# AbbVie-ComputationalGenomics/SAIGEgds

Hardware: AMD Instinct MI355X
Metric: variants/sec seqAssocGLMM_SPA at N=430K; achieved HBM GB/s vs roofline (higher is better)
Workload: dtype f64

## Files before the change

### saigegds_amd/csrc/host_init.h

```cpp
extern "C" const char *sgx_version(void) { return "saigehip 0.1 (gfx950)"; }
extern "C" const char *sgx_last_error(void) { return g_err.c_str(); }

extern "C" int sgx_device_count(void)
{
	int n = 0;
	if (hipGetDeviceCount(&n) != hipSuccess) return 0;
	return n;
}

extern "C" size_t sgx_row_stride(int32_t n_samp)
{
	return (size_t)((n_samp + 511) / 512) * 128;
}

static double thr_or(double v, double dflt) { return std::isfinite(v) ? v : dflt; }

extern "C" int sgx_set_thresholds(sgx_handle *h, double maf, double mac, double missing,
	double spa_pval)
{
	if (!h) return fail(SGX_EINVAL, "sgx_set_thresholds: NULL handle");
	h->md.thr_maf = thr_or(maf, -1);
	h->md.thr_mac = thr_or(mac, -1);
	h->md.thr_missing = thr_or(missing, 1);
	h->md.thr_spa = thr_or(spa_pval, 0.05);
// ... 61 lines not shown
			worst = std::max(worst, fabsl(t - (LD)m->t_XVX_inv_XV[(size_t)i * K + k]));
			scale = std::max(scale, fabsl((LD)m->t_XVX_inv_XV[(size_t)i * K + k]));
		}
	}
	if (!(worst <= 1e-13L * scale)) return false;
	for (int a = 0; a < K; a++)
		for (int b = 0; b < K; b++) out[(size_t)b * K + a] = (double)M[(size_t)a * K + b];
	for (int a = 0; a < K * K; a++) if (!std::isfinite(out[a])) return false;
	return true;
}

static int alloc_workspace(sgx_handle *h)
{
	const int N = h->md.N;
	{
		int least = 0, greatest = 0;
		HIPCHK(hipDeviceGetStreamPriorityRange(&least, &greatest));
		HIPCHK(h->stream.create(hipStreamNonBlocking, least));
		HIPCHK(h->hstream.create(hipStreamNonBlocking, greatest));
		HIPCHK(h->s3_side.create(hipStreamNonBlocking, greatest));
	}
	HIPCHK(h->s3_fork.create(hipEventDisableTiming));
	HIPCHK(h->s3_join.create(hipEventDisableTiming));
	HIPCHK(h->counters.alloc(24));
	HIPCHK(h->h_counters.alloc(24));
	for (DevEvent &e : h->ev) HIPCHK(e.create());
	for (DevEvent &e : h->evk) HIPCHK(e.create());
	HIPCHK(h->ev_lists.create());
	hipDeviceProp_t prop;
	HIPCHK(hipGetDeviceProperties(&prop, h->device));
	h->spa_grid = prop.multiProcessorCount * 2;
	h->n_cu = prop.multiProcessorCount;
	h->scratch_stride = 2 * (((size_t)N + 63) & ~(size_t)63);
	HIPCHK(h->scratch.alloc(h->scratch_stride * h->spa_grid));
	if (!h->md.quant) {
		h->nwg5 = ((size_t)((N + 63) / 64) * 16 <= 32 * 1024) ? h->n_cu * 4 : h->n_cu;
		HIPCHK(h->scr5.alloc((size_t)h->nwg5 * spa5_wg_bytes(N)));
		HIPCHK(h->cur5.alloc(8));
	}
	return SGX_OK;
}

static int check_model_consistency(const sgx_model *m)
{
	const int N = m->n_samp, K = m->n_coeff;
	if (!m->t_XXVX_inv || !m->XV)
		return fail(SGX_EINVAL, "sgx_init: SAIGEHIP_CHECK_MODEL needs t_XXVX_inv and XV");
	for (int i = 0; i < N; i++) {
		const double *x = m->t_X + (size_t)i * K, *xv = m->XV + (size_t)i * K,
			*a = m->t_XXVX_inv + (size_t)i * K, *av = m->t_XVX_inv_XV + (size_t)i * K;
		int k0 = 0;
		double sx = 0, sa = 0;
		for (int k = 0; k < K; k++) {
			if (std::fabs(x[k]) > std::fabs(x[k0])) k0 = k;
			sx = std::max(sx, std::fabs(xv[k])); sa = std::max(sa, std::fabs(av[k]));
		}
		if (x[k0] == 0) continue;
		const double V = xv[k0] / x[k0];
		for (int k = 0; k < K; k++) {
			if (std::fabs(xv[k] - V * x[k]) > 1e-8 * sx)
				return fail(SGX_EINVAL, "sgx_init: XV[%d,%d] = %g is not V t_X = %g", k, i, xv[k], V * x[k]);
			if (std::fabs(av[k] - V * a[k]) > 1e-8 * sa)
// ... 183 lines not shown
{
	if (!h) return;
	(void)hipSetDevice(h->device);
	for (hipStream_t st : {(hipStream_t)h->stream, (hipStream_t)h->s3_side, (hipStream_t)h->hstream}) if (st) (void)hipStreamSynchronize(st);
	for (sgx_handle *t : h->twins) sgx_free(t);
	for (sgx_block *b : h->tmp_blk) sgx_block_free(b);
	delete h;
}

static int ensure_recs(sgx_handle *h, size_t n)
{
	if (3 * n <= h->recs.cap) return SGX_OK;
	HIPCHK(hipStreamSynchronize(h->stream));
	HIPCHK(h->recs.release());
	int rc = grow(h->fallback, n);
	if (!rc && !h->md.quant) {
		h->nseg = (h->md.N + spa_seg(h->md.K) - 1) / spa_seg(h->md.K);
		rc = grow(h->fb_spa2, n);
		if (!rc) rc = grow(h->fb_x2, n);
		h->vcap4 = (int)std::min<size_t>(n, 65536);
		h->nround4 = (int)((n + h->vcap4 - 1) / h->vcap4);
		if (!rc) rc = grow(h->seg4, (size_t)h->nseg * SPA4_NSMAX * h->vcap4);
	}
	if (!rc && h->mf_ok) rc = grow(h->mf_acc, n * (size_t)(2 * h->mfe.acc_stride - 16));
	if (!rc) rc = grow(h->recs, 3 * n);
	return rc;
}
```

### saigegds_amd/csrc/host_scan.h

```cpp

template <typename T>
static int ensure_buf(sgx_handle *lane, DevBuf<T> &buf, size_t need)
{
	if (need <= buf.cap) return SGX_OK;
	for (hipStream_t st : {(hipStream_t)lane->stream, (hipStream_t)lane->hstream, (hipStream_t)lane->s3_side}) if (st) HIPCHK(hipStreamSynchronize(st));
	return grow(buf, need);
}

struct S3Shape { int nbf, naf, nc, nla, nlb, da, db; };
#define S3_SHAPE(...) S3Shape{__VA_ARGS__},
static constexpr S3Shape s3_shapes[2][15] = {{S3_FOR_EACH_NBF(S3_SHAPE)}, {S3_FOR_EACH_NBF_MISS(S3_SHAPE)}};
#undef S3_SHAPE

template <bool MISS, int I>
static int launch_score3(sgx_handle *h, const sgx_block *b, RowsRef rr, size_t M, int grid, int slots, S3Plan &pl)
{
	constexpr S3Shape s = s3_shapes[MISS][I];
	hipStream_t st = h->hstream;
	pl = s3_plan(M, b->ntile, grid, s.naf * s.nc, rr.bpv);
	int rc = ensure_buf(h, h->s3_slabs, (size_t)pl.ng * pl.ipg * s.nc * s.naf * slots * 256);
	if (rc) return rc;
	const size_t lds = s3_lds_bytes(s.nbf, s.naf, s.nc, s.da, s.db);
	auto kern = score3_kernel<s.nbf, s.naf, s.nc, s.nla, s.nlb, s.da, s.db, MISS>;
	bool &attr = (MISS ? h->s3_attr_miss : h->s3_attr)[s.nbf];
// ... 39 lines not shown
			const unsigned chunks = (unsigned)((M + 4 * tpw - 1) / (4 * tpw));
			hipLaunchKernelGGL(s3_t3_kernel<decltype(pp)::value>, dim3(chunks * (unsigned)b->nr), dim3(256), 0, h->s3_side,
				(int)M, md.P, h->dQ, L, h->s3_t3);
		});
		HIPCHK(hipGetLastError());
		HIPCHK(hipEventRecord(h->s3_join, h->s3_side));
		HIPCHK(hipStreamWaitEvent(st, h->s3_join, 0));
	}
	const bool miss = form == FORM_THREE;
	const int NBF = h->mf_nbfv[0] + 1;
	const int slots = miss ? 2 * NBF - 1 : NBF;
	const int grid = std::max(8, h->n_cu & ~7);
	constexpr int NSHAPE = (int)(sizeof s3_shapes[0] / sizeof s3_shapes[0][0]);
	int i = 0;
	while (i < NSHAPE && s3_shapes[miss][i].nbf != NBF) i++;
	S3Plan pl{};
	const auto shapes = std::make_integer_sequence<int, NSHAPE>();
	const bool found = miss ? with_int<0>(i, [&](auto I) { rc = launch_score3<true, decltype(I)::value>(h, b, rr, M, grid, slots, pl); }, shapes)
		: with_int<0>(i, [&](auto I) { rc = launch_score3<false, decltype(I)::value>(h, b, rr, M, grid, slots, pl); }, shapes);
	if (!found) return fail(SGX_EINVAL, "score3: %d B fragments not supported", NBF);
	if (rc) return rc;
	HIPCHK(hipGetLastError());
	const S3Shape &sh = s3_shapes[miss][i];
	const int acc_stride = 16 * slots;
	const int per = sh.nc * sh.naf * slots * 256;
	hipLaunchKernelGGL(s3_reduce_kernel, dim3((unsigned)((per / 4 + 255) / 256), (unsigned)pl.vt), dim3(256), 0, st,
		pl, (int)M, sh.nc, sh.naf, slots, h->s3_slabs, h->mf_acc, acc_stride, h->counters, h->cur5);
	const int btop = md.quant ? 0 : (int)(2 * M);
	if (!with_k(md.K, [&](auto kk) {
		constexpr int KK = decltype(kk)::value;
		hipLaunchKernelGGL((score3_epilogue<KK>), dim3((unsigned)((M + s3e_vb(KK) - 1) / s3e_vb(KK))), dim3(s3e_vb(KK)), 0, st,
			(int)M, md, h->mfe, h->mf_acc, acc_stride, miss ? 16 * NBF : 0, h->s3_t3, b->nr, L.lcnt, L.ld, h->s3_ovf, h->recs,
			h->counters, btop, h->fb_spa2, h->fb_x2, out8, valid, h->guard_tol);
		hipLaunchKernelGGL((score2b_kernel<2 * KK + 2, 256>), dim3((unsigned)std::min<size_t>(M, 4 * (size_t)h->n_cu)), dim3(256), 0, st,
			rr, (int)M, md, h->recs, h->counters, out8, valid, (const int *)h->s3_ovf, 23, btop, h->fb_spa2, h->fb_x2);
	}))
		return fail(SGX_EINVAL, "score3: unsupported K=%d", md.K);
	HIPCHK(hipGetLastError());
	return scan_end<IN_2BIT>(h, st, b, rr, M, out8, lazy_dense);
}

static int next_lane(sgx_handle *h, size_t M, sgx_handle **lane_out)
{
	sgx_handle *lane = h, *other = nullptr;
	if (h->n_lanes > 1) {
		lane = h->next_lane ? h->twins[h->next_lane - 1] : h;
		other = h->last_issued;
		h->next_lane = (h->next_lane + 1) % h->n_lanes;
	}
	int rc = sync_lane(lane);
	if (rc) return rc;
	h->last_issued = lane;
	rc = ensure_recs(lane, M);
	if (rc) return rc;
	if (other && other != lane && other->stats_pending) HIPCHK(hipStreamWaitEvent(lane->hstream, other->ev[1], 0));
	*lane_out = lane;
	return SGX_OK;
}

static int scan_form(const sgx_handle *lane, const sgx_block *b, ScanForm *form)
{
	const sgx_handle *p = lane->owner ? lane->owner : lane;
// ... 77 lines not shown
```

### saigegds_amd/csrc/host_spa.h

```cpp


template <int LO, typename F, int... I>
static bool with_int(int v, F &&f, std::integer_sequence<int, I...>)
{
	return ((v == LO + I && (f(std::integral_constant<int, LO + I>()), true)) || ...);
}
template <typename F>
static bool with_k(int K, F &&f) { return with_int<1>(K, f, std::make_integer_sequence<int, KMAX>()); }
template <typename F>
static void with_pp(int P, F &&f)
{
	if (P <= 8) f(std::integral_constant<int, 8>());
	else if (P <= 16) f(std::integral_constant<int, 16>());
	else if (P <= 32) f(std::integral_constant<int, 32>());
	else f(std::integral_constant<int, 64>());
}

static dim3 mf_grid(int n_cu, size_t rows, int ntile, int *tps, int vpb = MF_VPB, int wg_per_cu = 2)
{
	const int vt = (int)((rows + vpb - 1) / vpb);
	int sk = std::max(1, (n_cu * wg_per_cu * 4 + vt / 2) / vt);
	sk = std::min(sk, std::max(1, ntile / 24));
	if (sk >= 6) sk = (sk + 7) & ~7;
	sk = std::min(sk, std::max(1, ntile / 2));
	*tps = (ntile + sk - 1) / sk;
	*tps += *tps & 1;
	sk = (ntile + *tps - 1) / *tps;
	return dim3((unsigned)vt, (unsigned)sk);
}

template <int KK, int NCX, int INPUT>
static const void *spa4_moments_fn()
{
	if constexpr (INPUT == IN_2BIT) return (const void *)spa4_moments<KK, NCX>;
	else return (const void *)spa4_moments_ds<KK, NCX, INPUT>;
}

template <int KK, int INPUT>
static void launch_dense(sgx_handle *h, RowsRef rr, size_t M, int slot, const int *list, double *out8)
{
	const dim3 sgrid((unsigned)std::min<size_t>(M, (size_t)h->spa_grid));
	hipLaunchKernelGGL((spa_kernel<KK, 512, INPUT>), sgrid, dim3(512), 0, h->stream, rr,
		h->md, h->recs, h->counters, slot, list, h->scratch, h->scratch_stride, out8);
}

template <int KK, int INPUT>
static int launch_spa_k(sgx_handle *h, RowsRef rr, size_t M, double *out8, bool lazy_dense)
{
	const DevModel &md = h->md;
	hipStream_t st = h->stream;
	if (h->force_v1 && INPUT != IN_2BIT) {
		launch_dense<KK, INPUT>(h, rr, M, 0, nullptr, out8);
		return SGX_OK;
	}
	const size_t fl = spa4_lds_bytes(KK);
	if (!h->mom_attr_set[INPUT]) {
		HIPCHK(hipFuncSetAttribute(spa4_moments_fn<KK, SPA4_NCA, INPUT>(), hipFuncAttributeMaxDynamicSharedMemorySize, (int)fl));
		HIPCHK(hipFuncSetAttribute(spa4_moments_fn<KK, SPA4_NCB, INPUT>(), hipFuncAttributeMaxDynamicSharedMemorySize, (int)fl));
		h->mom_attr_set[INPUT] = true;
	}
	const int nround = (int)((M + h->vcap4 - 1) / h->vcap4);
	const int btop = (int)(2 * M);
	const dim3 gsolve((unsigned)std::min((h->vcap4 + 3) / 4, 4 * h->n_cu));
	const size_t rowb5 = (size_t)((md.N + 63) / 64) * 16;
	const size_t l5 = (INPUT == IN_2BIT && rowb5 <= 120 * 1024) ? rowb5 : 0;
	const bool small5 = INPUT == IN_2BIT && rowb5 <= 32 * 1024;
	if (l5 > 48 * 1024 && !h->spa5_attr_set[INPUT]) {
		HIPCHK(hipFuncSetAttribute((const void *)spa5_kernel<KK, INPUT, 0, 512>, hipFuncAttributeMaxDynamicSharedMemorySize, (int)l5));
		HIPCHK(hipFuncSetAttribute((const void *)spa5_kernel<KK, INPUT, 1, 512>, hipFuncAttributeMaxDynamicSharedMemorySize, (int)l5));
		h->spa5_attr_set[INPUT] = true;
	}
	auto moments = [&](auto ncx, int tier, int rd) {
		constexpr int NCX = decltype(ncx)::value;
		if constexpr (INPUT == IN_2BIT)
			hipLaunchKernelGGL((spa4_moments<KK, NCX>), dim3((unsigned)h->n_cu), dim3(WAVE * spa4_waves(KK)), fl, st, rr, md, h->nseg,
				tier, btop, rd * h->vcap4, h->vcap4, h->recs, h->counters, h->seg4, h->cur5 + 2);
		else
			hipLaunchKernelGGL((spa4_moments_ds<KK, NCX, INPUT>), dim3((unsigned)h->n_cu), dim3(WAVE * spa4_waves(KK)), fl, st,
				(const void *)rr.base, rr.bpv, md, h->nseg, tier, btop, rd * h->vcap4, h->vcap4, h->recs, h->counters, h->seg4, h->cur5 + 2);
		hipLaunchKernelGGL((spa4_solve<KK, NCX>), gsolve, dim3(256), 0, st, md, h->nseg, tier, btop, rd * h->vcap4, h->vcap4,
			h->recs, h->counters, h->seg4, h->fallback, h->fb_x2, out8, h->force_dense ? 1 : 0, h->force_exact ? 1 : 0);
	};
	for (int rd = 0; rd < nround; rd++) moments(std::integral_constant<int, SPA4_NCA>(), 0, rd);
	for (int rd = 0; rd < nround; rd++) moments(std::integral_constant<int, SPA4_NCB>(), 1, rd);
	const size_t ws5 = spa5_wg_bytes(md.N);
	auto spa5 = [&](auto threads, int nwg) {
		constexpr int T5 = decltype(threads)::value;
		if constexpr (T5 == 512 || INPUT == IN_2BIT) {
			hipLaunchKernelGGL((spa5_kernel<KK, INPUT, 0, T5>), dim3((unsigned)nwg), dim3(T5), l5, st, rr, md, h->recs, h->counters,
				h->fb_spa2, h->fb_x2, h->cur5, h->fallback, h->scr5, out8, h->force_dense ? 1 : 0, h->force_exact ? 1 : 0, l5,
				h->spa_scan_rows, ws5, 3);
			hipLaunchKernelGGL((spa5_kernel<KK, INPUT, 1, T5>), dim3((unsigned)nwg), dim3(T5), l5, st, rr, md, h->recs, h->counters,
				h->fb_x2, h->fb_x2, h->cur5 + 1, h->fallback, h->scr5, out8, h->force_dense ? 1 : 0, h->force_exact ? 1 : 0, l5,
				h->spa_scan_rows, ws5, 4);
		}
	};
	if (small5) spa5(std::integral_constant<int, 128>(), h->nwg5);
	else spa5(std::integral_constant<int, 512>(), h->n_cu);
	if (!lazy_dense) launch_dense<KK, INPUT>(h, rr, M, 2, h->fallback, out8);
	return SGX_OK;
}

template <int INPUT>
static int launch_spa(sgx_handle *h, RowsRef rr, size_t M, double *out8, bool lazy_dense = false)
{
	h->stats.spa_launches = 0;
	if (h->md.quant) return SGX_OK;
	int rc = SGX_OK;
	with_k(h->md.K, [&](auto kk) { rc = launch_spa_k<decltype(kk)::value, INPUT>(h, rr, M, out8, lazy_dense); });
	if (rc) return rc;
	HIPCHK(hipGetLastError());
	const bool v1 = h->force_v1 && INPUT != IN_2BIT;
	h->stats.spa_launches = v1 ? 1u : (uint32_t)(4 * ((M + h->vcap4 - 1) / h->vcap4) + 3);
	if (lazy_dense && !v1) { h->pend_dense.active = true; h->pend_dense.rr = rr; h->pend_dense.M = M; h->pend_dense.out8 = out8; }
	return SGX_OK;
}

static int launch_pending_dense(sgx_handle *h)
{
	with_k(h->md.K, [&](auto kk) {
		launch_dense<decltype(kk)::value, IN_2BIT>(h, h->pend_dense.rr, h->pend_dense.M, 2, h->fallback, h->pend_dense.out8);
	});
	HIPCHK(hipGetLastError());
	return SGX_OK;
}

static int scan_begin(sgx_handle *h, hipStream_t sst, ScanForm form, const sgx_block *b)
{
	h->form = form;
	if (b) HIPCHK(hipStreamWaitEvent(sst, b->ready, 0));
	if (form == FORM_FP64) {
		HIPCHK(hipMemsetAsync(h->counters, 0, 24 * sizeof(int), sst));
		if (h->cur5) HIPCHK(hipMemsetAsync(h->cur5, 0, 8 * sizeof(int), sst));
	}
	HIPCHK(hipEventRecord(h->ev[0], sst));
	return SGX_OK;
}

template <int INPUT>
static int scan_end(sgx_handle *h, hipStream_t sst, const sgx_block *b, RowsRef rr, size_t M, double *out8, bool lazy_dense)
{
	HIPCHK(hipEventRecord(h->ev[1], sst));
	h->stats.score_launches = h->form == FORM_FP64 ? 1 : 5;
	if (sst != h->stream) HIPCHK(hipStreamWaitEvent(h->stream, h->ev[1], 0));
	int rc = launch_spa<INPUT>(h, rr, M, out8, lazy_dense);
	if (rc) return rc;
	if (lazy_dense) h->pend_dense.blk = b;
	HIPCHK(hipEventRecord(h->ev[2], h->stream));
	if (b) {
		HIPCHK(hipEventRecord(b->last_read, h->stream));
		const_cast<sgx_block *>(b)->was_read = true;
	}
	HIPCHK(hipMemcpyAsync(h->h_counters, h->counters, 24 * sizeof(int), hipMemcpyDeviceToHost, h->stream));
	h->stats.n_variants = M;
	h->stats_pending = true;
	return SGX_OK;
}
// ... 51 lines not shown
```

### saigegds_amd/csrc/host_state.h

```cpp

struct sgx_block {
	int device = 0;
	int N = 0, ntile = 0, nr = 1;
	size_t cap = 0;
	size_t M = 0;
	bool lists_only = false;
	DevEvent ready;
	DevEvent last_read;
	bool was_read = false;
	DevBuf<uint8_t> rows;
	size_t bpv = 0;
	const uint8_t *ext_rows = nullptr; size_t ext_bpv = 0;
	DevBuf<unsigned> idx; size_t idx_cap = 0;
	DevBuf<unsigned> cursor;
	DevBuf<unsigned> lstart;
	DevBuf<int> lcnt;
	DevBuf<int> nzp, n2p;
	DevBuf<int> n3;
	DevBuf<uint8_t> ovf;
	DevBuf<int> nzv, n2v;
	DevBuf<unsigned> cptr;
	DevBuf<unsigned> cidx;
	size_t cidx_cap = 0;
	DevBuf<uint8_t> corient;
// ... 13 lines not shown
	DevStream stream;
	DevStream hstream;
	DevStream s3_side;
	DevStream cstream;
	DevEvent s3_fork, s3_join;
	DevEvent ev[3];
	DevEvent evk[2];
	DevEvent ev_lists;
	DevEvent ev_h2d;
	DevEvent ev_copy[2];
	DevEvent ev_done[2];
	struct { DevBuf<double> F, X, y, mu, mu2, XM; DevBuf<uint8_t> Fl; DevBuf<long long> Q; } model;
	DevModel md{};
	DevBuf<SpaRec> recs;
	DevBuf<int> fallback;
	DevBuf<int> fb_spa2;
	DevBuf<int> fb_x2;
	int nseg = 0;
	bool force_dense = false;
	DevBuf<double> seg4;
	int vcap4 = 0, nround4 = 0;
	bool spa5_attr_set[3] = {false, false, false};
	bool mom_attr_set[3] = {false, false, false};
	DevBuf<uint8_t> scr5; DevBuf<int> cur5; int nwg5 = 0;
	bool spa_scan_rows = false;
	bool force_exact = false;
	bool mf_ok = false;
	MfTab mf[MF_MAXG]{};
	int mf_nbfv[MF_MAXG]{};
	MfEpi mfe{};
	const long long *dQ = nullptr;
	DevBuf<int> mf_acc;
	DevBuf<int> s3_slabs;
	DevBuf<long long> s3_t3;
	DevBuf<int> s3_ovf;
	bool s3_attr[17] = {false};
	bool s3_attr_miss[17] = {false};
	sgx_block *tmp_blk[2] = {nullptr, nullptr};
	int n_cu = 256;
	DevBuf<int> counters;
	PinBuf<int> h_counters;
	DevBuf<double> scratch; size_t scratch_stride = 0; int spa_grid = 0;
	DevBuf<uint8_t> stage_in;
	size_t pipe_bytes = 0;
	DevBuf<uint8_t> pipe_in[2];
	DevBuf<uint8_t> pipe_raw[2];
	DevBuf<uint8_t> pipe_pk[2];
	DevBuf<int> pipe_flag; PinBuf<int> h_pipe_flag;
	DevBuf<int> pk_sel;
	DevBuf<unsigned> db2_row0;
	DevBuf<double> pipe_out[2]; DevBuf<uint8_t> pipe_valid[2];
	PinBuf<double> pin_out[2]; PinBuf<uint8_t> pin_valid[2];
	DevBuf<uint8_t> stage_pk;
	DevBuf<double> ds_part;
	DevBuf<double> skat_part;
	DevBuf<double> skat_fin;
	DevBuf<double> stage_out; DevBuf<uint8_t> stage_valid;
	DevBuf<double> skk_A, skk_Y, skk_XZ, skk_cpart, skk_cs;
	DevBuf<SkkTile> skk_tiles;
	double skk_ms[3] = {0, 0, 0};
	DevBuf<double> ckm_set;
	int ckm_n = 0;
	sgx_kmat *ckm_km = nullptr;
	std::vector<double> ckm_D, ckm_q, ckm_Einv, ckm_w;
	std::vector<uint8_t> ckm_bad;
	bool ckm_eok = false;
	double ckm_tau[2] = {0, 0}, ckm_tol = 0;
	int ckm_maxiter = 0;
	DevBuf<double> cond_B;
	DevBuf<double> cond_ce;
	int n_cond = 0;
	DevBuf<double> cond_part, cond_fin;
	DevBuf<uint8_t> firth_scr;
	DevBuf<double> eig_A, eig_out, eig_scr;
	DevBuf<int> eig_sw;
	DevBuf<uint8_t> eig_meta;
	bool eig_attr_set = false;
	bool evk_set = false;
	bool lists_timed = false;
	sgx_stats stats{};
	bool force_v1 = false;
	bool stats_pending = false;
	struct { bool active = false; RowsRef rr{}; size_t M = 0; double *out8 = nullptr; const sgx_block *blk = nullptr; } pend_dense;
	sgx_handle *twins[3] = {nullptr, nullptr, nullptr};
	int n_lanes = 1;
	sgx_handle *owner = nullptr;
	bool dense_mode = false;
	int dense_opt = -1;
	double guard_tol = 2e-11;
	ScanForm form = FORM_FP64;
	int next_lane = 0;
	sgx_handle *last_issued = nullptr;
	sgx_stats total{};
	uint64_t total_calls = 0;
};

#define SGX_DENSE_ON  0.005
#define SGX_DENSE_OFF 0.003

static int set_dev(sgx_handle *h)
{
	HIPCHK(hipSetDevice(h->device));
	return SGX_OK;
}
```

### saigegds_amd/csrc/kern_score.h

```cpp
#pragma once


template <int P, int BLOCK>
__global__ void __launch_bounds__(BLOCK)
score2b_kernel(RowsRef rr, int M, DevModel md,
	SpaRec *__restrict__ recs, int *__restrict__ counters, double *__restrict__ out8,
	uint8_t *__restrict__ valid, const int *__restrict__ list, int list_counter, int btop, int *__restrict__ fb_series, int *__restrict__ fb_exact)
{
	__shared__ double sh[P * (BLOCK / WAVE)];
	__shared__ int shi[3 * (BLOCK / WAVE)];
	const int nwork = list ? counters[list_counter] : M;
	for (int wi = blockIdx.x; wi < nwork; wi += gridDim.x) {
	const int j = list ? list[wi] : wi;
	const int N = md.N, tid = threadIdx.x;
	const int lane = tid & (WAVE - 1), wid = tid / WAVE;
	constexpr int NW = BLOCK / WAVE;
	const int nvec = (N + 63) >> 6;
	auto row_piece = [&](int v) -> uint4 { return *reinterpret_cast<const uint4 *>(rr.base + rr_piece(rr, (size_t)j, (size_t)v)); };
	__syncthreads();

	int n1 = 0, n2 = 0, n3 = 0;
	for (int v = tid; v < nvec; v += BLOCK) {
		const uint4 q = row_piece(v);
		const uint32_t ww[4] = {q.x, q.y, q.z, q.w};
#pragma unroll
		for (int d = 0; d < 4; d++) {
			const uint32_t w = ww[d] & keep_mask(N - (v * 64 + d * 16));
			const uint32_t lo = w & LO_MASK, hi = (w >> 1) & LO_MASK;
			n3 += __popc(lo & hi);
			n1 += __popc(lo & ~hi);
			n2 += __popc(hi & ~lo);
		}
	}
	n1 = wave_sum_i(n1); n2 = wave_sum_i(n2); n3 = wave_sum_i(n3);
	if (lane == 0) { shi[wid] = n1; shi[NW + wid] = n2; shi[2 * NW + wid] = n3; }
	__syncthreads();
	n1 = n2 = n3 = 0;
#pragma unroll
	for (int w = 0; w < NW; w++) { n1 += shi[w]; n2 += shi[NW + w]; n3 += shi[2 * NW + w]; }

	const VarHead h = make_head(md, double(n1 + 2 * n2), N - n3);
	if (!h.pass) {
		if (tid == 0) { nan_row(out8 + (size_t)j * 8); valid[j] = 0; }
		continue;
	}

	double acc[P];
#pragma unroll
	for (int a = 0; a < P; a++) acc[a] = 0;
	const uint32_t zx = h.minus ? 0xAAAAAAAAu : 0u;
	const double *__restrict__ F = md.F;
	for (int v = tid; v < nvec; v += BLOCK) {
		const uint4 q = row_piece(v);
		const uint32_t ww[4] = {q.x, q.y, q.z, q.w};
#pragma unroll
		for (int d = 0; d < 4; d++) {
			const int base = v * 64 + d * 16;
			const uint32_t km = keep_mask(N - base);
			const uint32_t w = ww[d];
			uint32_t nz = nz_fields((w ^ zx) & km) ;
			while (nz) {
				const int b = __ffs(nz) - 1;
				nz &= nz - 1;
				const double g = sel4(h.lut, (w >> b) & 3u);
				const double *f = F + (size_t)(base + (b >> 1)) * P;
#pragma unroll
				for (int a = 0; a < P - 2; a += 2) {
					const double2 t = *reinterpret_cast<const double2 *>(f + a);
					acc[a] = fma(g, t.x, acc[a]);
					acc[a + 1] = fma(g, t.y, acc[a + 1]);
				}
				const double2 t = *reinterpret_cast<const double2 *>(f + P - 2);
				acc[P - 2] = fma(g, t.x, acc[P - 2]);
				acc[P - 1] = fma(g * g, t.y, acc[P - 1]);
			}
		}
	}
	block_sum<P, BLOCK>(acc, sh);

	if (tid == 0) {
		double *o = out8 + (size_t)j * 8;
		double cbuf[KMAX], pn, Ssc, v2sc;
		valid[j] = 1;
		if (score_epilogue<(P - 2) / 2>(md, h, acc, o, cbuf, &pn, &Ssc, &v2sc)) {
			spa_push<(P - 2) / 2>(md, recs, counters, btop, fb_series, fb_exact, j, h.minus, h.minus ? (2 * h.Num - h.AC) : h.AC,
				h.minus ? (N - n2) : (n1 + n2 + n3), h.lut, pn, Ssc, v2sc, cbuf);
		}
		atomicAdd(&counters[1], 1);
	}
	}
}


template <typename T> __device__ __forceinline__ bool ds_missing(T v);
template <> __device__ __forceinline__ bool ds_missing<uint8_t>(uint8_t v) { return v == 0xFF; }
template <> __device__ __forceinline__ bool ds_missing<double>(double v) { return !isfinite(v); }

template <int P, int BLOCK, typename T>
__global__ void __launch_bounds__(BLOCK)
score_ds_kernel(const T *__restrict__ ds, int M, DevModel md, SpaRec *__restrict__ recs,
	int *__restrict__ counters, double *__restrict__ out8, uint8_t *__restrict__ valid)
{
	__shared__ double sh[P * (BLOCK / WAVE)];
	const int j = blockIdx.x;
	if (j >= M) return;
	const int N = md.N, tid = threadIdx.x;
	const T *row = ds + (size_t)j * N;

	double hd[2] = {0, 0};
	for (int i = tid; i < N; i += BLOCK) {
		const T v = row[i];
		if (!ds_missing<T>(v)) { hd[0] += (double)v; hd[1] += 1.0; }
	}
// ... 157 lines not shown
```

### saigegds_amd/csrc/kern_score3.h

```cpp
#pragma once
#include <type_traits>

#ifndef S3_V4I_DEFINED
#define S3_V4I_DEFINED
typedef int s3_v4i __attribute__((ext_vector_type(4)));
#endif

#include "s3_layout.h"

template <int OFF> __device__ __forceinline__ void s3_ds_read(s3_v4i &dst, uint32_t addr)
{
	asm volatile("ds_read_b128 %0, %1 offset:%2" : "=v"(dst) : "v"(addr), "n"(OFF));
}
template <int N> __device__ __forceinline__ void s3_lgkm_wait(s3_v4i &reg) { asm volatile("s_waitcnt lgkmcnt(%1)" : "+v"(reg) : "n"(N)); }
__device__ __forceinline__ void s3_tie(s3_v4i &reg) { asm volatile("" : "+v"(reg)); }
template <int N, int CNT> __device__ __forceinline__ void s3_wait_regs(s3_v4i *regs)
{
	s3_lgkm_wait<N>(regs[0]);
#pragma unroll
	for (int i = 1; i < CNT; i++) s3_tie(regs[i]);
}

template <int I, int N, typename F>
__device__ __forceinline__ void s3_static_for(F &&f)
// ... 507 lines not shown
		for (int k = 0; k < NB; k++) mine[k] = (e + k * PP + c < e1) ? idx[e + k * PP + c] : 0xFFFFFFFFu;
		constexpr int UN = PP <= 16 ? 8 : 4;
		constexpr int UNR = PP <= 16 ? 2 : 1;
#pragma unroll
		for (int k = 0; k < NB; k++)
#pragma unroll UNR
			for (int j0 = 0; j0 < PP; j0 += UN) {
				long long q[UN];
#pragma unroll
				for (int j = 0; j < UN; j++) {
					const unsigned s = (unsigned)__shfl((int)mine[k], gbase + j0 + j, 64);
					q[j] = (s != 0xFFFFFFFFu && c < P) ? Q[(size_t)s * P + c] : 0;
				}
#pragma unroll
				for (int j = 0; j < UN; j++) { hi += q[j] >> 32; lo += q[j] & 0xFFFFFFFFll; }
			}
	}
	if (v < M && c < P) {
		long long *o = part + (((size_t)g * M + v) * P + c) * 2;
		o[0] = hi; o[1] = lo;
	}
}

__global__ void __launch_bounds__(256)
s3_reduce_kernel(S3Plan pl, int M, int NC, int NAF, int NBF, const int *__restrict__ slabs, int *__restrict__ accbuf, int stride,
	int *__restrict__ counters, int *__restrict__ cursors)
{
	if (blockIdx.x == 0 && blockIdx.y == 0 && threadIdx.x < 32) {
		if (threadIdx.x < 24) counters[threadIdx.x] = 0;
		if (threadIdx.x < 8 && cursors) cursors[threadIdx.x] = 0;
	}
	const int e = (blockIdx.x * 256 + threadIdx.x) * 4, per = NC * NAF * NBF * 256, vtile = blockIdx.y;
	if (e >= per) return;
	const int lane = e & 63, reg = (e >> 6) & 3, fb = e >> 8;
	const int b = fb % NBF, wf = fb / NBF;
	const int v = (vtile * pl.fpw + wf) * 16 + (lane >> 4) * 4 + reg;
	if (v >= M) return;
	s3_v4i sum = (s3_v4i){0, 0, 0, 0};
	for (int g = 0; g < pl.ng; g++) {
		int first, count;
		s3_items_of(pl, vtile, g, first, count);
		for (int id = first; id < first + count; id++) sum += *reinterpret_cast<const s3_v4i *>(slabs + (size_t)id * per + e);
	}
	*reinterpret_cast<s3_v4i *>(accbuf + (size_t)v * stride + b * 16 + (lane & 15)) = sum;
}

__host__ __device__ constexpr int s3e_vb(int K) { return K <= 8 ? 256 : 128; }
template <int K>
__global__ void __launch_bounds__(256)
score3_epilogue(int M, DevModel md, MfEpi ep, const int *__restrict__ accbuf, int acc_stride, int miss_off,
	const long long *__restrict__ t3part , int nr,
	const int *__restrict__ lcnt , size_t ld, int *__restrict__ ovf_list,
	SpaRec *__restrict__ recs, int *__restrict__ counters, int btop, int *__restrict__ fb_series, int *__restrict__ fb_exact,
	double *__restrict__ out8, uint8_t *__restrict__ valid, double guard_tol)
{
	constexpr int P = 2 * K + 2, CW = P - 1;
	constexpr int S3E_VB = s3e_vb(K);
	__shared__ double s_acc[S3E_VB][P | 1];
	__shared__ double s_imp[S3E_VB];
	__shared__ int s_n[S3E_VB][4];
	__shared__ long long s_ftot[P][2];
	__shared__ int s_col[P][3];
	const int tid = threadIdx.x, j0 = blockIdx.x * S3E_VB;
	const int N = md.N;
	for (int c = tid; c < P; c += S3E_VB) {
		s_col[c][0] = ep.ccol[c]; s_col[c][1] = ep.climb[c]; s_col[c][2] = ep.escale[c];
		s_ftot[c][0] = ep.ftot_hi[c]; s_ftot[c][1] = ep.ftot_lo[c];
	}
	{
		const int j = j0 + tid;
		const int *a0 = accbuf + (size_t)min(j, M - 1) * acc_stride;
		int n3 = 0;
		bool over = false;
		if (miss_off) n3 = a0[miss_off + ep.col_ones] / 4;
		else {
			for (int g0 = 0; g0 < nr; g0 += 8) {
				int cn[8];
#pragma unroll
				for (int u = 0; u < 8; u++) cn[u] = lcnt[(size_t)min(g0 + u, nr - 1) * ld + min(j, M - 1)];
#pragma unroll
				for (int u = 0; u < 8; u++) if (g0 + u < nr) { over |= cn[u] < 0; n3 += cn[u] < 0 ? 0 : cn[u]; }
			}
		}
		if (j >= M) n3 = 0;
		{
			const int tot = wave_total_i(n3);
			if ((tid & 63) == 0 && tot >= 64) atomicAdd(&counters[22], tot >> 6);
		}
		int state = 0, n1 = 0, n2 = 0;
		double imp = 0;
		if (j < M) {
			if (over) ovf_list[atomicAdd(&counters[23], 1)] = j;
			else {
				const long long AC = (long long)(a0[ep.col_ones] / 4) - 3ll * n3;
				n2 = a0[ep.col_b1 + ep.climb[CW]] / 8 - n3;
				n1 = (int)(AC - 2ll * n2);
				const VarHead h = make_head(md, (double)AC, N - n3);
				if (!h.pass) { nan_row(out8 + (size_t)j * 8); valid[j] = 0; }
				else { state = h.minus ? 2 : 1; imp = 2 * h.AF; }
			}
		}
		s_n[tid][0] = n1; s_n[tid][1] = n2; s_n[tid][2] = n3; s_n[tid][3] = state;
		s_imp[tid] = imp;
	}
	__syncthreads();
	for (int task = tid; task < S3E_VB * P; task += S3E_VB) {
		const int vl = task / P, c = task - vl * P, j = j0 + vl;
		const int state = s_n[vl][3];
		if (!state) continue;
		const int cc = s_col[c][0], nl = s_col[c][1];
		if (nl == 0) { s_acc[vl][c] = 0; continue; }
		const int *a0 = accbuf + (size_t)j * acc_stride;
		const bool minus = state == 2;
		const double imp = s_imp[vl];
		int lv[MF_NLIMB], lm[MF_NLIMB], lb[MF_NLIMB];
#pragma unroll
		for (int l = 0; l < MF_NLIMB; l++) lv[l] = a0[cc + min(l, nl - 1)];
		HiLo T3 = hl(0, 0);
		if (miss_off) {
#pragma unroll
			for (int l = 0; l < MF_NLIMB; l++) lm[l] = a0[miss_off + cc + min(l, nl - 1)];
		} else {
			const long long *p = t3part + ((size_t)j * P + c) * 2;
			const size_t gs = (size_t)M * P * 2;
			for (int g0 = 0; g0 < nr; g0 += 8) {
				long long ph[8], pl[8];
#pragma unroll
				for (int u = 0; u < 8; u++) { const long long *q = p + (size_t)min(g0 + u, nr - 1) * gs; ph[u] = q[0]; pl[u] = q[1]; }
#pragma unroll
				for (int u = 0; u < 8; u++) if (g0 + u < nr) { T3.hi += ph[u]; T3.lo += pl[u]; }
			}
		}
		if (c == CW) {
#pragma unroll
			for (int l = 0; l < MF_NLIMB; l++) lb[l] = a0[ep.col_b1 + min(l, nl - 1)];
		}
		auto limbs = [&](const int (&x)[MF_NLIMB]) -> HiLo {
			long long lo = 0, hi = 0;
#pragma unroll
			for (int l = 3; l >= 0; l--) lo = lo * 256 + (l < nl ? x[l] : 0);
#pragma unroll
			for (int l = MF_NLIMB - 1; l >= 4; l--) hi = hi * 256 + (l < nl ? x[l] : 0);
			return hl(hi, lo);
		};
		const HiLo V = limbs(lv);
		if (miss_off) T3 = limbs(lm);
		const HiLo W = hl_axpy(-3, T3, V);
		const double t3d = hl_to_double(T3);
		double r;
		if (c != CW) {
			double sm;
			if (!minus) sm = hl_to_double(W) + imp * t3d;
			else sm = hl_to_double(hl(2 * s_ftot[c][0] - W.hi, 2 * s_ftot[c][1] - W.lo)) - imp * t3d;
			r = ldexp(sm, -s_col[c][2]);
		} else {
			const HiLo B2 = limbs(lb);
			const HiLo H2 = hl(B2.hi / 2 - T3.hi, B2.lo / 2 - T3.lo);
			double w;
			if (!minus) {
				w = hl_to_double(hl_axpy(2, H2, W)) + imp * imp * t3d;
			} else {
				const HiLo S1 = hl_axpy(-2, H2, W);
				const HiLo R = hl(s_ftot[CW][0] - S1.hi - H2.hi - T3.hi, s_ftot[CW][1] - S1.lo - H2.lo - T3.lo);
				w = hl_to_double(hl_axpy(4, R, S1)) + (2 - imp) * (2 - imp) * t3d;
			}
			r = ldexp(w, -s_col[CW][2]);
		}
		s_acc[vl][c] = r;
	}
	__syncthreads();
	const int j = j0 + tid;
	if (j >= M || !s_n[tid][3]) return;
	const int n1 = s_n[tid][0], n2 = s_n[tid][1], n3 = s_n[tid][2];
	const long long AC = (long long)n1 + 2ll * n2;
	const VarHead h = make_head(md, (double)AC, N - n3);
	const double imp = 2 * h.AF;
	double *o = out8 + (size_t)j * 8;
	double acc[P];
#pragma unroll
	for (int c = 0; c < P; c++) acc[c] = s_acc[tid][c];
	if (ep.derive_c) {
#pragma unroll
		for (int x = 0; x < K; x++) {
			double cx = 0;
#pragma unroll
			for (int y = 0; y < K; y++) cx = fma(ep.XVXi[x * K + y], acc[K + y], cx);
			acc[x] = cx;
		}
	}
	{
		const double g2 = (double)n1 + 4.0 * n2 + (h.minus ? (2 - imp) * (2 - imp) : imp * imp) * n3;
		const double spread = 8.0 * sqrt(fmax(g2, 1.0));
		double dcol[P];
#pragma unroll
		for (int c = 0; c < P; c++) dcol[c] = (ep.climb[c] && !(md.quant && c == CW)) ? spread * ldexp(1.0, -ep.escale[c]) : 0.0;
// ... 6 lines not shown
			sat[y] = t;
		}
		double dquad = 0, dec = 0, dS = dcol[2 * K], quad = 0, ec = 0, sac = 0;
#pragma unroll
		for (int a = 0; a < K; a++) {
			double t = 0;
#pragma unroll
			for (int b = 0; b < K; b++) t = fma(md.XVX[a * K + b], acc[b], t);
			quad = fma(t, acc[a], quad);
			dquad += 2 * dcol[a] * fabs(t - acc[K + a]);
			ec = fma(acc[K + a], acc[a], ec);
			dec += dcol[K + a] * fabs(acc[a]);
			sac = fma(md.S_a[a], acc[a], sac);
			dS += ep.derive_c ? fabs(sat[a]) * dcol[K + a] : fabs(md.S_a[a]) * dcol[a];
		}
		const double var2 = quad + acc[CW] - 2 * ec, S = acc[2 * K] - sac;
		const double dvar = dquad + 2 * dec + dcol[CW];
		const double sd = sqrt(md.r * fmax(var2, 0.0) * (md.quant ? 1.0 / fmax(h.mac, 1.0) : 1.0)) * (md.quant ? md.tau0 * sqrt(fmax(h.mac, 1.0)) : 1.0);
		const double z = fabs(S) / sd;
		const double dz = dS / sd + 0.5 * z * dvar / var2;
		if (!(dz * fmax(1.0, z) <= guard_tol)) {
			ovf_list[atomicAdd(&counters[23], 1)] = j;
			atomicAdd(&counters[21], 1);
			return;
		}
	}
	double cbuf[KMAX], pn, Ssc, v2sc;
	valid[j] = 1;
	if (score_epilogue<(P - 2) / 2>(md, h, acc, o, cbuf, &pn, &Ssc, &v2sc)) {
		spa_push<K>(md, recs, counters, btop, fb_series, fb_exact, j, h.minus, h.minus ? (2 * h.Num - h.AC) : h.AC,
			h.minus ? (N - n2) : (n1 + n2 + n3), h.lut, pn, Ssc, v2sc, cbuf);
	}
	{
		const unsigned long long act = __ballot(true);
		if (__builtin_amdgcn_mbcnt_hi((uint32_t)(act >> 32), __builtin_amdgcn_mbcnt_lo((uint32_t)act, 0u)) == 0u) atomicAdd(&counters[1], (int)__popcll(act));
	}
}
#endif
```

Baseline: 18.51 million.

## Fuse slab reduction, epilogue and overflow fallback into one score3 tail kernel

```diff
diff --git a/saigegds_amd/csrc/host_init.h b/saigegds_amd/csrc/host_init.h
--- a/saigegds_amd/csrc/host_init.h
+++ b/saigegds_amd/csrc/host_init.h
@@ -107,7 +107,9 @@
 	}
 	HIPCHK(h->s3_fork.create(hipEventDisableTiming));
 	HIPCHK(h->s3_join.create(hipEventDisableTiming));
-	HIPCHK(h->counters.alloc(24));
+	HIPCHK(h->cnt_sets.alloc(2 * 24));
+	HIPCHK(hipMemsetAsync(h->cnt_sets, 0, 2 * 24 * sizeof(int), h->stream));
+	h->counters = h->cnt_sets; h->cset = 0; h->sets_clean = false;
 	HIPCHK(h->h_counters.alloc(24));
 	for (DevEvent &e : h->ev) HIPCHK(e.create());
 	for (DevEvent &e : h->evk) HIPCHK(e.create());
@@ -121,8 +123,12 @@
 	if (!h->md.quant) {
 		h->nwg5 = ((size_t)((N + 63) / 64) * 16 <= 32 * 1024) ? h->n_cu * 4 : h->n_cu;
 		HIPCHK(h->scr5.alloc((size_t)h->nwg5 * spa5_wg_bytes(N)));
-		HIPCHK(h->cur5.alloc(8));
-	}
+		HIPCHK(h->cur_sets.alloc(2 * 8));
+		HIPCHK(hipMemsetAsync(h->cur_sets, 0, 2 * 8 * sizeof(int), h->stream));
+		h->cur5 = h->cur_sets;
+	}
+	HIPCHK(hipStreamSynchronize(h->stream));
+	h->sets_clean = true;
 	return SGX_OK;
 }
 
@@ -352,7 +358,6 @@
 		h->nround4 = (int)((n + h->vcap4 - 1) / h->vcap4);
 		if (!rc) rc = grow(h->seg4, (size_t)h->nseg * SPA4_NSMAX * h->vcap4);
 	}
-	if (!rc && h->mf_ok) rc = grow(h->mf_acc, n * (size_t)(2 * h->mfe.acc_stride - 16));
 	if (!rc) rc = grow(h->recs, 3 * n);
 	return rc;
 }
diff --git a/saigegds_amd/csrc/host_scan.h b/saigegds_amd/csrc/host_scan.h
--- a/saigegds_amd/csrc/host_scan.h
+++ b/saigegds_amd/csrc/host_scan.h
@@ -85,22 +85,29 @@
 	if (rc) return rc;
 	HIPCHK(hipGetLastError());
 	const S3Shape &sh = s3_shapes[miss][i];
-	const int acc_stride = 16 * slots;
-	const int per = sh.nc * sh.naf * slots * 256;
-	hipLaunchKernelGGL(s3_reduce_kernel, dim3((unsigned)((per / 4 + 255) / 256), (unsigned)pl.vt), dim3(256), 0, st,
-		pl, (int)M, sh.nc, sh.naf, slots, h->s3_slabs, h->mf_acc, acc_stride, h->counters, h->cur5);
+	int *const next_counters = h->cnt_sets + 24 * (h->cset ^ 1);
+	int *const next_cursors = h->cur_sets ? h->cur_sets + 8 * (h->cset ^ 1) : nullptr;
 	const int btop = md.quant ? 0 : (int)(2 * M);
+	const size_t tlds = s3t_lds_bytes(md.K, slots);
 	if (!with_k(md.K, [&](auto kk) {
 		constexpr int KK = decltype(kk)::value;
-		hipLaunchKernelGGL((score3_epilogue<KK>), dim3((unsigned)((M + s3e_vb(KK) - 1) / s3e_vb(KK))), dim3(s3e_vb(KK)), 0, st,
-			(int)M, md, h->mfe, h->mf_acc, acc_stride, miss ? 16 * NBF : 0, h->s3_t3, b->nr, L.lcnt, L.ld, h->s3_ovf, h->recs,
-			h->counters, btop, h->fb_spa2, h->fb_x2, out8, valid, h->guard_tol);
-		hipLaunchKernelGGL((score2b_kernel<2 * KK + 2, 256>), dim3((unsigned)std::min<size_t>(M, 4 * (size_t)h->n_cu)), dim3(256), 0, st,
-			rr, (int)M, md, h->recs, h->counters, out8, valid, (const int *)h->s3_ovf, 23, btop, h->fb_spa2, h->fb_x2);
+		if (!h->s3t_attr) {
+			(void)hipFuncSetAttribute((const void *)score3_tail<KK>, hipFuncAttributeMaxDynamicSharedMemorySize, 48 * 1024);
+			h->s3t_attr = true;
+		}
+		hipLaunchKernelGGL((score3_tail<KK>), dim3((unsigned)((M + s3e_vb(KK) - 1) / s3e_vb(KK))), dim3(s3e_vb(KK)), tlds, st,
+			(int)M, md, h->mfe, pl, sh.nc, sh.naf, slots, s3t_fps(KK, slots), (const int *)h->s3_slabs, miss ? 16 * NBF : 0,
+			h->s3_t3, b->nr, L.lcnt, L.ld, h->s3_ovf, h->recs, h->counters, next_counters, next_cursors, btop, h->fb_spa2, h->fb_x2,
+			out8, valid, h->guard_tol, rr);
 	}))
 		return fail(SGX_EINVAL, "score3: unsupported K=%d", md.K);
 	HIPCHK(hipGetLastError());
-	return scan_end<IN_2BIT>(h, st, b, rr, M, out8, lazy_dense);
+	rc = scan_end<IN_2BIT>(h, st, b, rr, M, out8, lazy_dense);
+	if (rc) return rc;
+	h->cset ^= 1;
+	h->counters = next_counters; h->cur5 = next_cursors;
+	h->sets_clean = true;
+	return SGX_OK;
 }
 
 static int next_lane(sgx_handle *h, size_t M, sgx_handle **lane_out)
diff --git a/saigegds_amd/csrc/host_spa.h b/saigegds_amd/csrc/host_spa.h
--- a/saigegds_amd/csrc/host_spa.h
+++ b/saigegds_amd/csrc/host_spa.h
@@ -37,11 +37,11 @@
 }
 
 template <int KK, int INPUT>
-static void launch_dense(sgx_handle *h, RowsRef rr, size_t M, int slot, const int *list, double *out8)
+static void launch_dense(sgx_handle *h, RowsRef rr, size_t M, int slot, const int *list, double *out8, int *counters)
 {
 	const dim3 sgrid((unsigned)std::min<size_t>(M, (size_t)h->spa_grid));
 	hipLaunchKernelGGL((spa_kernel<KK, 512, INPUT>), sgrid, dim3(512), 0, h->stream, rr,
-		h->md, h->recs, h->counters, slot, list, h->scratch, h->scratch_stride, out8);
+		h->md, h->recs, counters, slot, list, h->scratch, h->scratch_stride, out8);
 }
 
 template <int KK, int INPUT>
@@ -50,7 +50,7 @@
 	const DevModel &md = h->md;
 	hipStream_t st = h->stream;
 	if (h->force_v1 && INPUT != IN_2BIT) {
-		launch_dense<KK, INPUT>(h, rr, M, 0, nullptr, out8);
+		launch_dense<KK, INPUT>(h, rr, M, 0, nullptr, out8, h->counters);
 		return SGX_OK;
 	}
 	const size_t fl = spa4_lds_bytes(KK);
@@ -97,7 +97,7 @@
 	};
 	if (small5) spa5(std::integral_constant<int, 128>(), h->nwg5);
 	else spa5(std::integral_constant<int, 512>(), h->n_cu);
-	if (!lazy_dense) launch_dense<KK, INPUT>(h, rr, M, 2, h->fallback, out8);
+	if (!lazy_dense) launch_dense<KK, INPUT>(h, rr, M, 2, h->fallback, out8, h->counters);
 	return SGX_OK;
 }
 
@@ -112,14 +112,14 @@
 	HIPCHK(hipGetLastError());
 	const bool v1 = h->force_v1 && INPUT != IN_2BIT;
 	h->stats.spa_launches = v1 ? 1u : (uint32_t)(4 * ((M + h->vcap4 - 1) / h->vcap4) + 3);
-	if (lazy_dense && !v1) { h->pend_dense.active = true; h->pend_dense.rr = rr; h->pend_dense.M = M; h->pend_dense.out8 = out8; }
+	if (lazy_dense && !v1) { h->pend_dense.active = true; h->pend_dense.rr = rr; h->pend_dense.M = M; h->pend_dense.out8 = out8; h->pend_dense.counters = h->counters; }
 	return SGX_OK;
 }
 
 static int launch_pending_dense(sgx_handle *h)
 {
 	with_k(h->md.K, [&](auto kk) {
-		launch_dense<decltype(kk)::value, IN_2BIT>(h, h->pend_dense.rr, h->pend_dense.M, 2, h->fallback, h->pend_dense.out8);
+		launch_dense<decltype(kk)::value, IN_2BIT>(h, h->pend_dense.rr, h->pend_dense.M, 2, h->fallback, h->pend_dense.out8, h->pend_dense.counters);
 	});
 	HIPCHK(hipGetLastError());
 	return SGX_OK;
@@ -129,10 +129,11 @@
 {
 	h->form = form;
 	if (b) HIPCHK(hipStreamWaitEvent(sst, b->ready, 0));
-	if (form == FORM_FP64) {
+	if (form == FORM_FP64 || !h->sets_clean) {
 		HIPCHK(hipMemsetAsync(h->counters, 0, 24 * sizeof(int), sst));
 		if (h->cur5) HIPCHK(hipMemsetAsync(h->cur5, 0, 8 * sizeof(int), sst));
 	}
+	h->sets_clean = false;
 	HIPCHK(hipEventRecord(h->ev[0], sst));
 	return SGX_OK;
 }
diff --git a/saigegds_amd/csrc/host_state.h b/saigegds_amd/csrc/host_state.h
--- a/saigegds_amd/csrc/host_state.h
+++ b/saigegds_amd/csrc/host_state.h
@@ -59,7 +59,7 @@
 	int vcap4 = 0, nround4 = 0;
 	bool spa5_attr_set[3] = {false, false, false};
 	bool mom_attr_set[3] = {false, false, false};
-	DevBuf<uint8_t> scr5; DevBuf<int> cur5; int nwg5 = 0;
+	DevBuf<uint8_t> scr5; int nwg5 = 0;
 	bool spa_scan_rows = false;
 	bool force_exact = false;
 	bool mf_ok = false;
@@ -67,15 +67,19 @@
 	int mf_nbfv[MF_MAXG]{};
 	MfEpi mfe{};
 	const long long *dQ = nullptr;
-	DevBuf<int> mf_acc;
 	DevBuf<int> s3_slabs;
 	DevBuf<long long> s3_t3;
 	DevBuf<int> s3_ovf;
 	bool s3_attr[17] = {false};
 	bool s3_attr_miss[17] = {false};
+	bool s3t_attr = false;
 	sgx_block *tmp_blk[2] = {nullptr, nullptr};
 	int n_cu = 256;
-	DevBuf<int> counters;
+	DevBuf<int> cnt_sets, cur_sets;
+	int *counters = nullptr;
+	int *cur5 = nullptr;
+	int cset = 0;
+	bool sets_clean = false;
 	PinBuf<int> h_counters;
 	DevBuf<double> scratch; size_t scratch_stride = 0; int spa_grid = 0;
 	DevBuf<uint8_t> stage_in;
@@ -118,7 +122,7 @@
 	sgx_stats stats{};
 	bool force_v1 = false;
 	bool stats_pending = false;
-	struct { bool active = false; RowsRef rr{}; size_t M = 0; double *out8 = nullptr; const sgx_block *blk = nullptr; } pend_dense;
+	struct { bool active = false; RowsRef rr{}; size_t M = 0; double *out8 = nullptr; const sgx_block *blk = nullptr; int *counters = nullptr; } pend_dense;
 	sgx_handle *twins[3] = {nullptr, nullptr, nullptr};
 	int n_lanes = 1;
 	sgx_handle *owner = nullptr;
diff --git a/saigegds_amd/csrc/kern_score.h b/saigegds_amd/csrc/kern_score.h
--- a/saigegds_amd/csrc/kern_score.h
+++ b/saigegds_amd/csrc/kern_score.h
@@ -2,16 +2,10 @@
 
 
 template <int P, int BLOCK>
-__global__ void __launch_bounds__(BLOCK)
-score2b_kernel(RowsRef rr, int M, DevModel md,
+__device__ __forceinline__ void score2b_variant(const RowsRef &rr, int j, const DevModel &md,
 	SpaRec *__restrict__ recs, int *__restrict__ counters, double *__restrict__ out8,
-	uint8_t *__restrict__ valid, const int *__restrict__ list, int list_counter, int btop, int *__restrict__ fb_series, int *__restrict__ fb_exact)
-{
-	__shared__ double sh[P * (BLOCK / WAVE)];
-	__shared__ int shi[3 * (BLOCK / WAVE)];
-	const int nwork = list ? counters[list_counter] : M;
-	for (int wi = blockIdx.x; wi < nwork; wi += gridDim.x) {
-	const int j = list ? list[wi] : wi;
+	uint8_t *__restrict__ valid, int btop, int *__restrict__ fb_series, int *__restrict__ fb_exact, double *sh, int *shi)
+{
 	const int N = md.N, tid = threadIdx.x;
 	const int lane = tid & (WAVE - 1), wid = tid / WAVE;
 	constexpr int NW = BLOCK / WAVE;
@@ -42,7 +36,7 @@
 	const VarHead h = make_head(md, double(n1 + 2 * n2), N - n3);
 	if (!h.pass) {
 		if (tid == 0) { nan_row(out8 + (size_t)j * 8); valid[j] = 0; }
-		continue;
+		return;
 	}
 
 	double acc[P];
@@ -88,7 +82,19 @@
 		}
 		atomicAdd(&counters[1], 1);
 	}
-	}
+}
+
+template <int P, int BLOCK>
+__global__ void __launch_bounds__(BLOCK)
+score2b_kernel(RowsRef rr, int M, DevModel md,
+	SpaRec *__restrict__ recs, int *__restrict__ counters, double *__restrict__ out8,
+	uint8_t *__restrict__ valid, const int *__restrict__ list, int list_counter, int btop, int *__restrict__ fb_series, int *__restrict__ fb_exact)
+{
+	__shared__ double sh[P * (BLOCK / WAVE)];
+	__shared__ int shi[3 * (BLOCK / WAVE)];
+	const int nwork = list ? counters[list_counter] : M;
+	for (int wi = blockIdx.x; wi < nwork; wi += gridDim.x)
+		score2b_variant<P, BLOCK>(rr, list ? list[wi] : wi, md, recs, counters, out8, valid, btop, fb_series, fb_exact, sh, shi);
 }
 
 
diff --git a/saigegds_amd/csrc/kern_score3.h b/saigegds_amd/csrc/kern_score3.h
--- a/saigegds_amd/csrc/kern_score3.h
+++ b/saigegds_amd/csrc/kern_score3.h
@@ -553,58 +553,53 @@
 	}
 }
 
-__global__ void __launch_bounds__(256)
-s3_reduce_kernel(S3Plan pl, int M, int NC, int NAF, int NBF, const int *__restrict__ slabs, int *__restrict__ accbuf, int stride,
-	int *__restrict__ counters, int *__restrict__ cursors)
-{
-	if (blockIdx.x == 0 && blockIdx.y == 0 && threadIdx.x < 32) {
-		if (threadIdx.x < 24) counters[threadIdx.x] = 0;
-		if (threadIdx.x < 8 && cursors) cursors[threadIdx.x] = 0;
-	}
-	const int e = (blockIdx.x * 256 + threadIdx.x) * 4, per = NC * NAF * NBF * 256, vtile = blockIdx.y;
-	if (e >= per) return;
-	const int lane = e & 63, reg = (e >> 6) & 3, fb = e >> 8;
-	const int b = fb % NBF, wf = fb / NBF;
-	const int v = (vtile * pl.fpw + wf) * 16 + (lane >> 4) * 4 + reg;
-	if (v >= M) return;
-	s3_v4i sum = (s3_v4i){0, 0, 0, 0};
-	for (int g = 0; g < pl.ng; g++) {
-		int first, count;
-		s3_items_of(pl, vtile, g, first, count);
-		for (int id = first; id < first + count; id++) sum += *reinterpret_cast<const s3_v4i *>(slabs + (size_t)id * per + e);
-	}
-	*reinterpret_cast<s3_v4i *>(accbuf + (size_t)v * stride + b * 16 + (lane & 15)) = sum;
-}
-
-__host__ __device__ constexpr int s3e_vb(int K) { return K <= 8 ? 256 : 128; }
+#ifndef S3E_VB
+#define S3E_VB 128
+#endif
+__host__ __device__ constexpr int s3e_vb(int K) { return S3E_VB; }
+static inline int s3t_fps(int K, int slots)
+{
+	const int vf = s3e_vb(K) / 16, most = 28 / slots < 1 ? 1 : 28 / slots;
+	const int nsub = (vf + most - 1) / most;
+	return (vf + nsub - 1) / nsub;
+}
+__host__ __device__ constexpr int s3t_stride(int slots) { return 16 * slots + 4; }
+static inline size_t s3t_lds_bytes(int K, int slots) { return (size_t)s3t_fps(K, slots) * 16 * s3t_stride(slots) * sizeof(int); }
 template <int K>
-__global__ void __launch_bounds__(256)
-score3_epilogue(int M, DevModel md, MfEpi ep, const int *__restrict__ accbuf, int acc_stride, int miss_off,
+__global__ void __launch_bounds__(S3E_VB)
+score3_tail(int M, DevModel md, MfEpi ep, S3Plan pl, int NC, int NAF, int slots, int fps, const int *__restrict__ slabs, int miss_off,
 	const long long *__restrict__ t3part , int nr,
 	const int *__restrict__ lcnt , size_t ld, int *__restrict__ ovf_list,
-	SpaRec *__restrict__ recs, int *__restrict__ counters, int btop, int *__restrict__ fb_series, int *__restrict__ fb_exact,
-	double *__restrict__ out8, uint8_t *__restrict__ valid, double guard_tol)
+	SpaRec *__restrict__ recs, int *__restrict__ counters, int *__restrict__ next_counters, int *__restrict__ next_cursors,
+	int btop, int *__restrict__ fb_series, int *__restrict__ fb_exact,
+	double *__restrict__ out8, uint8_t *__restrict__ valid, double guard_tol, RowsRef rr)
 {
 	constexpr int P = 2 * K + 2, CW = P - 1;
-	constexpr int S3E_VB = s3e_vb(K);
+	constexpr int VF = S3E_VB / 16;
+	extern __shared__ __attribute__((aligned(16))) int s_stage[];
 	__shared__ double s_acc[S3E_VB][P | 1];
 	__shared__ double s_imp[S3E_VB];
 	__shared__ int s_n[S3E_VB][4];
+	__shared__ int s_fp[S3E_VB];
 	__shared__ long long s_ftot[P][2];
 	__shared__ int s_col[P][3];
+	__shared__ double s_sh[P * (S3E_VB / WAVE)];
+	__shared__ int s_shi[3 * (S3E_VB / WAVE)];
 	const int tid = threadIdx.x, j0 = blockIdx.x * S3E_VB;
 	const int N = md.N;
 	for (int c = tid; c < P; c += S3E_VB) {
 		s_col[c][0] = ep.ccol[c]; s_col[c][1] = ep.climb[c]; s_col[c][2] = ep.escale[c];
 		s_ftot[c][0] = ep.ftot_hi[c]; s_ftot[c][1] = ep.ftot_lo[c];
 	}
+	if (blockIdx.x == 0 && tid < 32) {
+		if (tid < 24) next_counters[tid] = 0;
+		if (tid < 8 && next_cursors) next_cursors[tid] = 0;
+	}
 	{
 		const int j = j0 + tid;
-		const int *a0 = accbuf + (size_t)min(j, M - 1) * acc_stride;
 		int n3 = 0;
 		bool over = false;
-		if (miss_off) n3 = a0[miss_off + ep.col_ones] / 4;
-		else {
+		if (!miss_off) {
 			for (int g0 = 0; g0 < nr; g0 += 8) {
 				int cn[8];
 #pragma unroll
@@ -613,15 +608,41 @@
 				for (int u = 0; u < 8; u++) if (g0 + u < nr) { over |= cn[u] < 0; n3 += cn[u] < 0 ? 0 : cn[u]; }
 			}
 		}
-		if (j >= M) n3 = 0;
-		{
-			const int tot = wave_total_i(n3);
-			if ((tid & 63) == 0 && tot >= 64) atomicAdd(&counters[22], tot >> 6);
-		}
+		s_n[tid][2] = j < M ? n3 : 0;
+		s_fp[tid] = j < M && over;
+	}
+	const int fq = slots * 64, fsz = slots * 256, per = NC * NAF * fsz, lstride = s3t_stride(slots);
+	for (int fl0 = 0; fl0 < VF; fl0 += fps) {
+	const int nf = min(fps, VF - fl0);
+	for (int q = tid; q < nf * fq; q += S3E_VB) {
+		const int fl = q / fq, e = (q - fl * fq) * 4, fr = blockIdx.x * VF + fl0 + fl;
+		const int lane = e & 63, reg = (e >> 6) & 3, b = e >> 8, vi = (lane >> 4) * 4 + reg;
+		s3_v4i sum = (s3_v4i){0, 0, 0, 0};
+		if (fr * 16 + vi < M) {
+			const int vtile = fr / pl.fpw, wf = fr - vtile * pl.fpw;
+			int first, count;
+			s3_items_of(pl, vtile, 0, first, count);
+			const int *src = slabs + (size_t)wf * fsz + e;
+			for (int i = 0; i < count; i++) {
+				s3_v4i x[8];
+#pragma unroll
+				for (int u = 0; u < 8; u++) x[u] = *reinterpret_cast<const s3_v4i *>(src + ((size_t)min(u, pl.ng - 1) * pl.ipg + first + i) * per);
+#pragma unroll
+				for (int u = 0; u < 8; u++) if (u < pl.ng) sum += x[u];
+			}
+		}
+		*reinterpret_cast<s3_v4i *>(s_stage + (fl * 16 + vi) * lstride + b * 16 + (lane & 15)) = sum;
+	}
+	__syncthreads();
+	if (tid < nf * 16) {
+		const int vl = fl0 * 16 + tid, j = j0 + vl;
+		const int *a0 = s_stage + tid * lstride;
+		int n3 = s_n[vl][2];
+		if (miss_off) n3 = j < M ? a0[miss_off + ep.col_ones] / 4 : 0;
 		int state = 0, n1 = 0, n2 = 0;
 		double imp = 0;
 		if (j < M) {
-			if (over) ovf_list[atomicAdd(&counters[23], 1)] = j;
+			if (s_fp[vl]) ovf_list[atomicAdd(&counters[23], 1)] = j;
 			else {
 				const long long AC = (long long)(a0[ep.col_ones] / 4) - 3ll * n3;
 				n2 = a0[ep.col_b1 + ep.climb[CW]] / 8 - n3;
@@ -631,17 +652,17 @@
 				else { state = h.minus ? 2 : 1; imp = 2 * h.AF; }
 			}
 		}
-		s_n[tid][0] = n1; s_n[tid][1] = n2; s_n[tid][2] = n3; s_n[tid][3] = state;
-		s_imp[tid] = imp;
+		s_n[vl][0] = n1; s_n[vl][1] = n2; s_n[vl][2] = n3; s_n[vl][3] = state;
+		s_imp[vl] = imp;
 	}
 	__syncthreads();
-	for (int task = tid; task < S3E_VB * P; task += S3E_VB) {
-		const int vl = task / P, c = task - vl * P, j = j0 + vl;
+	for (int task = tid; task < nf * 16 * P; task += S3E_VB) {
+		const int vs = task / P, c = task - vs * P, vl = fl0 * 16 + vs, j = j0 + vl;
 		const int state = s_n[vl][3];
 		if (!state) continue;
 		const int cc = s_col[c][0], nl = s_col[c][1];
 		if (nl == 0) { s_acc[vl][c] = 0; continue; }
-		const int *a0 = accbuf + (size_t)j * acc_stride;
+		const int *a0 = s_stage + vs * lstride;
 		const bool minus = state == 2;
 		const double imp = s_imp[vl];
 		int lv[MF_NLIMB], lm[MF_NLIMB], lb[MF_NLIMB];
@@ -655,11 +676,11 @@
 			const long long *p = t3part + ((size_t)j * P + c) * 2;
 			const size_t gs = (size_t)M * P * 2;
 			for (int g0 = 0; g0 < nr; g0 += 8) {
-				long long ph[8], pl[8];
-#pragma unroll
-				for (int u = 0; u < 8; u++) { const long long *q = p + (size_t)min(g0 + u, nr - 1) * gs; ph[u] = q[0]; pl[u] = q[1]; }
-#pragma unroll
-				for (int u = 0; u < 8; u++) if (g0 + u < nr) { T3.hi += ph[u]; T3.lo += pl[u]; }
+				long long qh[8], ql[8];
+#pragma unroll
+				for (int u = 0; u < 8; u++) { const long long *q = p + (size_t)min(g0 + u, nr - 1) * gs; qh[u] = q[0]; ql[u] = q[1]; }
+#pragma unroll
+				for (int u = 0; u < 8; u++) if (g0 + u < nr) { T3.hi += qh[u]; T3.lo += ql[u]; }
 			}
 		}
 		if (c == CW) {
@@ -700,8 +721,13 @@
 		s_acc[vl][c] = r;
 	}
 	__syncthreads();
+	}
 	const int j = j0 + tid;
-	if (j >= M || !s_n[tid][3]) return;
+	{
+		const int tot = wave_total_i(s_n[tid][2]);
+		if ((tid & 63) == 0 && tot >= 64) atomicAdd(&counters[22], tot >> 6);
+	}
+	auto finish = [&]() {
 	const int n1 = s_n[tid][0], n2 = s_n[tid][1], n3 = s_n[tid][2];
 	const long long AC = (long long)n1 + 2ll * n2;
 	const VarHead h = make_head(md, (double)AC, N - n3);
@@ -754,6 +780,7 @@
 		if (!(dz * fmax(1.0, z) <= guard_tol)) {
 			ovf_list[atomicAdd(&counters[23], 1)] = j;
 			atomicAdd(&counters[21], 1);
+			s_fp[tid] = 1;
 			return;
 		}
 	}
@@ -767,5 +794,11 @@
 		const unsigned long long act = __ballot(true);
 		if (__builtin_amdgcn_mbcnt_hi((uint32_t)(act >> 32), __builtin_amdgcn_mbcnt_lo((uint32_t)act, 0u)) == 0u) atomicAdd(&counters[1], (int)__popcll(act));
 	}
+	};
+	if (j < M && s_n[tid][3]) finish();
+	if (!__syncthreads_or(s_fp[tid])) return;
+	for (int v = 0; v < S3E_VB; v++)
+		if (__builtin_amdgcn_readfirstlane(s_fp[v]))
+			score2b_variant<P, S3E_VB>(rr, j0 + v, md, recs, counters, out8, valid, btop, fb_series, fb_exact, s_sh, s_shi);
 }
 #endif
```

New measurement: 18.00 million. -2.8%, worse.
